# HpWang-whu/RoReg

Hardware: AMD Instinct MI355X
Metric: pair-registrations/sec (higher is better)
Workload: dtype f32 (every f32 operand enters the fp16 matrix cores as hi + lo fp16 under a per-keypoint power-of-two block scale: <= 22 significant bits relative to a CONSERVATIVE per-keypoint bound -- measured on the extractor: the bound sits 2^2..2^6 above the keypoint's true coefficient maximum (config.f16x2_sc

## Files before the change

include/roreg_hip.h:

```cpp
#ifndef ROREG_HIP_H
#define ROREG_HIP_H

#include <stdint.h>
#include <stddef.h>

#ifdef __cplusplus
extern "C" {
#endif

#define ROREG_ABI_VERSION 6
int roreg_abi_version(void);
const char *roreg_last_error(void);

int roreg_set_group_tables(const int32_t *P_host, const int32_t *Nei_host, const double *R_host);

size_t roreg_group_conv_packed_size(int Cin, int Cout, int KS);
int roreg_group_conv_pack_weights(const float *W_host , int Cin, int Cout, int KS,
                                  float *wpack_host );
size_t roreg_group_conv_workspace_size(int B, int Cin, int Cout, int Lin, int Lout, int KS);
int roreg_group_conv(const float *x, const float *wpack, const float *bias,
                     const float *bn_scale, const float *bn_shift, const float *residual,
                     float *out, const int32_t *gather,
                     int B, int Cin, int Cout, int Lin, int Lout, int KS,
                     float *workspace, size_t workspace_floats, void *stream);
// ... 217 lines not shown
int roreg_irrep_gemm(const float *const *X, float *const *Out, const float *const *Add, const float *const *Wpack, int C, int O, int B,
                     const int32_t *tiles_dev, int n_tiles, void *stream);
int roreg_irrep_gemm_split(const float *const *X, float *const *Out, const float *const *Add, const void *const *Wsplit, int C, int O, int B,
                           const int32_t *tiles_dev, int n_tiles, void *stream);
int roreg_irrep_gemm_f16x2(const float *const *X, float *const *Out, const float *const *Add, const void *const *Wsplit2,
                           const float *x_bound_dev, int w_exp, const float *next_u_dev, const float *next_v_dev, float *out_bound_dev,
                           int C, int O, int B, const int32_t *tiles_dev, int n_tiles,
                           int tile_m ,
                           int x_planes , void *stream);
int roreg_gemm_persistent(int on);
int roreg_gemm_thin(int on);
int roreg_irrep_gemm_f16x2_rows(const float *const *X, float *T3r, const void *const *Wsplit2, const float *x_bound_dev, int w_exp, int C, int B, void *stream);
int roreg_gf_finish(const float *T3r, const float *x, const float *b_out, const float *role_scale , const float *role_shift ,
                    float *eqv, float *inv, float *role_out , float *eqv_ft, int B, void *stream);
int roreg_gf_finish_route(int on);
int roreg_row_bound(const void *x_spatial, int x_bf16 , const float *bn_scale, const float *bn_shift,
                    float *bound_out, int B, int C, void *stream);
int roreg_ft_nonlin(const float *Xin , const float *x_spatial, const float *bias,
                    const float *bias2, const float *bn_scale, const float *bn_shift, const float *resid_spatial,
                    float *Xout , float *out_spatial ,
                    const int32_t *g_map ,
                    int Lout , int Lvalid,
                    int B, int C, int split ,
                    const float *out_bound ,
                    float *out_rowmax ,
                    int spatial_bf16 ,
                    int out_planes ,
                    void *stream);
int roreg_ft_nonlin_packed(const float *Xin, const float *bias, const float *bn_scale, const float *bn_shift, uint32_t *out_words,
                           const int32_t *g_map, int Lout, int Lvalid, int B, int C, const float *out_bound, float *raw_col, int raw_g,
// ... 210 lines not shown
```

roreg_amd/_abi.py:

```python
import ctypes
from ctypes import c_int, c_void_p, c_size_t, c_double, c_float, c_char_p

import numpy as np

ABI_VERSION = 6

_P = c_void_p
PROTOTYPES = {
    'roreg_abi_version': (c_int, []),
    'roreg_last_error': (c_char_p, []),
    'roreg_set_group_tables': (c_int, [_P, _P, _P]),
    'roreg_group_conv_packed_size': (c_size_t, [c_int, c_int, c_int]),
    'roreg_group_conv_pack_weights': (c_int, [_P, c_int, c_int, c_int, _P]),
    'roreg_group_conv_workspace_size': (c_size_t, [c_int, c_int, c_int, c_int, c_int, c_int]),
    'roreg_group_conv': (c_int, [_P, _P, _P, _P, _P, _P, _P, _P, c_int, c_int, c_int, c_int, c_int, c_int, _P, c_size_t, _P]),
    'roreg_group_conv_split': (c_int, [_P, _P, _P, _P, _P, _P, _P, _P, c_int, c_int, c_int, c_int, c_int, c_int, c_int, _P]),
    'roreg_group_conv_f16x2': (c_int, [_P, _P, c_int, _P, _P, _P, c_float, c_float, _P, _P, _P, _P, _P, c_int, c_int, c_int, c_int, c_int, c_int, c_int, _P]),
    'roreg_group_conv_f16x2_packed': (c_int, [_P, _P, c_int, _P, _P, _P, _P, _P, _P, c_int, c_int, c_int, c_int, c_int, c_int, c_int, _P]),
    'roreg_dense_f16x2': (c_int, [_P, _P, c_int, _P, _P, _P, c_float, c_float, _P, _P, c_int, _P, _P, c_int, c_int, c_int, _P]),
    'roreg_dense_split': (c_int, [_P, _P, _P, _P, _P, _P, c_int, _P, c_int, c_int, c_int, _P]),
    'roreg_gf_finalize': (c_int, [_P, _P, c_int, _P, c_int, _P]),
    'roreg_det_score': (c_int, [_P, _P, c_int, _P]),
    'roreg_inv_descriptor': (c_int, [_P, c_int, _P, c_int, _P]),
    'roreg_nn_search': (c_int, [_P, _P, c_int, _P, _P, c_int, c_int, _P, _P, _P, _P]),
# ... 42 lines not shown
    'roreg_sinkhorn_batch3_workspace_size': (c_size_t, [c_int, c_int, c_int, ctypes.c_longlong, ctypes.c_longlong, c_int, c_int]),
    'roreg_sinkhorn_batch3': (c_int, [_P, _P, _P, _P, _P, _P, _P, c_int, c_float, c_int, _P, _P, _P, _P, _P, c_size_t, c_int, _P, _P]),
    'roreg_write_files': (c_int, [_P, _P, _P, _P, _P, c_int, c_int]),
    'roreg_yohoc_draw_many': (c_int, [_P, c_int, _P, _P, c_int, c_int, _P, _P, _P, c_int]),
    'roreg_mlp_head_workspace': (c_size_t, [c_int, c_int, c_int]),
    'roreg_mlp_head': (c_int, [_P, _P, _P, _P, _P, c_int, c_int, c_int, c_int, _P, _P, c_int, _P, _P, _P, _P, _P, c_int, c_int, c_float, _P, _P, _P]),
    'roreg_sinkhorn_early_exit': (c_int, [c_int]),
    'roreg_sinkhorn_iteration_stats': (c_int, [_P, _P, c_int, _P]),
    'roreg_linear': (c_int, [_P, c_int, c_int, _P, _P, c_int, _P, _P]),
    'roreg_linear_mfma': (c_int, [_P, c_int, c_int, _P, _P, c_int, _P, _P]),
    'roreg_linear_path': (c_int, [c_int]),
    'roreg_linear_cat3': (c_int, [_P, _P, _P, _P, c_int, c_int, _P, _P, c_int, _P, _P]),
    'roreg_gemm_persistent': (c_int, [c_int]),
    'roreg_gemm_thin': (c_int, [c_int]),
    'roreg_gf_finish_route': (c_int, [c_int]),
    'roreg_irrep_gemm_f16x2_rows': (c_int, [_P, _P, _P, _P, c_int, c_int, c_int, _P]),
    'roreg_gf_finish': (c_int, [_P, _P, _P, _P, _P, _P, _P, _P, _P, c_int, _P]),
    'roreg_instnorm_stats': (c_int, [_P, c_int, c_int, c_float, _P, _P, _P, c_int, c_int, _P]),
    'roreg_mlp_tail': (c_int, [_P, c_int, c_int, _P, _P, _P, _P, _P, c_int, c_int, _P]),
    'roreg_mlp_tail_mfma': (c_int, [_P, c_int, c_int, _P, _P, _P, _P, _P, c_int, c_int, _P]),
    'roreg_knn_attention': (c_int, [_P, _P, _P, _P, c_int, c_int, c_int, c_int, _P, _P]),
    'roreg_rm_elementwise': (c_int, [c_int, _P, _P, _P, _P, c_int, c_int, c_int, _P, _P, _P]),
    'roreg_sinkhorn_workspace_size': (c_size_t, [c_int, c_int]),
    'roreg_sinkhorn': (c_int, [_P, c_int, _P, c_int, c_float, c_int, _P, _P, _P, _P, _P, _P, c_size_t, _P]),
    'roreg_icp_grid_size': (c_size_t, [_P, _P, c_int, c_double, _P, _P]),
    'roreg_icp_grid_build': (c_int, [_P, _P, _P, _P, c_size_t, _P]),
    'roreg_icp_batch_workspace': (c_size_t, [c_int, ctypes.c_longlong]),
    'roreg_icp_batch': (c_int, [_P, c_int, _P, c_int, ctypes.c_longlong, c_double, c_int, c_double, c_double, _P, _P, _P, _P, _P, _P, _P, _P, c_size_t, _P]),
    'roreg_icp_normals': (c_int, [_P, c_double, c_int, _P, _P]),
    'roreg_icp_plane_batch_workspace': (c_size_t, [c_int, ctypes.c_longlong]),
# ... 94 lines not shown
```

roreg_amd/_hip_fourier.py:

```python
import os
from ctypes import c_void_p

import numpy as np
import torch

from . import hip as _core
from .hip import HipError, _check, _feat, _ptr, _stream, lib

__all__ = ['DenseSplitLayer', 'IRREP_DIMS', 'IRREP_OFFSETS', '_bf16_split3', '_keypoint_of_columns', '_ptr_array', '_res_ptr', '_tile_cache', 'bf16_split3_frags', 'bf16_split3_pack', 'bound_exp', 'coef_pitch', 'coef_size', 'coef_views', 'dense_split', 'ensure_fourier', 'f16_scale_exp', 'f16_split2_frags', 'f16_split2_pack', 'frag_pack', 'ft_nonlin', 'ft_nonlin_gathered', 'ft_nonlin_packed', 'gemm_persistent', 'gemm_thin', 'gf_finish', 'gf_finish_rows', 'gf_finish_usable', 'group_conv_split_pack', 'irrep_gemm', 'irrep_gemm_rows', 'next_bound', 'next_bound_spatial', 'pack_coefs_f16x2', 'row_bound', 'unpack_coefs_f16x2', 'words_to_planes']


_fourier_ready = False
IRREP_DIMS = (1, 3, 3, 4, 5)
IRREP_OFFSETS = (0, 1, 10, 19, 35, 60)


def ensure_fourier():
    global _fourier_ready
    if not _fourier_ready:
        from .fourier import group_fourier
        F = np.ascontiguousarray(group_fourier().F, np.float32)
        _check(lib().roreg_set_fourier_tables(F.ctypes.data), 'roreg_set_fourier_tables')
        _fourier_ready = True

# ... 135 lines not shown
def row_bound(x, bn=None, roles=None):
    B, C = int(x.shape[0]), int(x.shape[1])
    out = torch.empty(coef_pitch(B), dtype=torch.float32, device=x.device)
    scale, shift = bn if bn is not None else (None, None)
    xp, bf = _feat(x)
    if roles is not None:
        if bn is not None or C != 32:
            raise HipError('row_bound: roles go with the 32-channel input features and no BatchNorm')
        r_scale, r_shift, role = _core._role_args(roles, B)
        _check(lib().roreg_row_bound_roles(xp, bf, _ptr(out), _ptr(r_scale), _ptr(r_shift), _ptr(role), B, _stream()), 'roreg_row_bound_roles')
        return out
    _check(lib().roreg_row_bound(xp, bf, _ptr(scale), _ptr(shift), _ptr(out), B, C, _stream()), 'roreg_row_bound')
    return out


def _keypoint_of_columns(d, Bp):
    n = torch.arange(d * Bp, device='cuda')
    return ((n // 32) // d) * 32 + (n % 32)


def bound_exp(bound):
    _, ex = torch.frexp(bound.float())
    e = torch.where((bound > 0) & torch.isfinite(bound), 14 - ex, torch.zeros_like(ex))
    return e.clamp(-100, 100)


def pack_coefs_f16x2(X_buf, C, B, bound=None):
    Bp = coef_pitch(B)
    views = coef_views(X_buf, C, B)
    if bound is None:
# ... 204 lines not shown
```

roreg_amd/csrc/fourier.hip:

```cpp
#include "common.h"
#include "primitives.h"
#include <algorithm>
#include <atomic>
#include <cmath>
#include <cstdlib>
#include <type_traits>
#include <utility>
#include <vector>

namespace {

constexpr int NIRR = 5;

struct GemmDescs {
    const float *X[NIRR];
    float *Out[NIRR];
    const float *Add[NIRR];
    const float4 *W[NIRR];
    int K[NIRR], M[NIRR], Mpad[NIRR], N[NIRR];
};

__device__ __forceinline__ void lds_dma16(const void *src, void *dst) {
    __builtin_amdgcn_global_load_lds((const __attribute__((address_space(1))) void *)src, (__attribute__((address_space(3))) void *)dst, 16, 0, 0);
}
// ... 1573 lines not shown
                t.qa[s] = off + l; t.row[s] = row0 + l; t.i[s] = 0; t.d[s] = d;
                if (l + 1 < d) { t.qb[s] = off + l + 1; t.kind[s] = 1; } else { t.qb[s] = 64; t.kind[s] = 2; }
            }
        off += d * d; row0 += d;
    }
    return t;
}
constexpr PairSlots kPS = make_pair_slots();
constexpr int slot_out_q(int m) { const int mm = m & 31, s = (m >> 5) * 16 + (mm & 3) + 4 * (mm >> 3); return (mm & 4) ? kPS.qb[s] : kPS.qa[s]; }

template <int... I, class F>
__device__ __forceinline__ void static_for_impl(std::integer_sequence<int, I...>, F &&f) { (f(std::integral_constant<int, I>{}), ...); }
template <int N, class F>
__device__ __forceinline__ void static_for(F &&f) { static_for_impl(std::make_integer_sequence<int, N>{}, f); }

template <bool IN_SPATIAL, bool OUT_SPATIAL, int SPLIT , int NW , int MINW , bool OUT_ROWS = false, bool GATHER = false >
__global__ __launch_bounds__(NW * 64, MINW) void ft_nonlin_kernel(NonlinParams p) {
    constexpr int NT = NW * 64;
    const int lane = threadIdx.x & 63;
    const int jn = lane & 31, h = lane >> 5;
    const int wave_global = __builtin_amdgcn_readfirstlane((blockIdx.x * NT + threadIdx.x) >> 6);
    const int n_waves = gridDim.x * NW;
    const int B = p.B, C = p.C;
    const int n_tiles = C * p.tiles_per_c;

    constexpr int NPL = SPLIT == 2 ? 2 : 3;
    constexpr int NA1 = SPLIT ? 4 * 2 * NPL * 64 * 4 : 30 * 2 * 64, NA2 = SPLIT ? 4 * 2 * NPL * 64 * 4 : 32 * 2 * 64;
    __shared__ __attribute__((aligned(16))) float sA1[IN_SPATIAL ? 64 : NA1];
    __shared__ __attribute__((aligned(16))) float sA2[OUT_SPATIAL ? 64 : NA2];
    __shared__ float sT[(IN_SPATIAL || OUT_SPATIAL || OUT_ROWS) ? NW * 32 * 65 : 64];
// ... 14 lines not shown
    for (int i = threadIdx.x; i < p.C; i += NT) {
        sBias[i] = (p.bias ? p.bias[i] : 0.f) + (p.bias2 ? p.bias2[i] : 0.f);
        sScale[i] = p.bn_scale ? p.bn_scale[i] : 1.f;
        sShift[i] = p.bn_shift ? p.bn_shift[i] : 0.f;
    }
    __syncthreads();
    const bf16x8 *sA1s = reinterpret_cast<const bf16x8 *>(sA1), *sA2s = reinterpret_cast<const bf16x8 *>(sA2);
    const f16x8 *sA1h = reinterpret_cast<const f16x8 *>(sA1), *sA2h = reinterpret_cast<const f16x8 *>(sA2);
    const size_t Bp = (size_t)p.Bp;
    const size_t hmask = (size_t)0 - (size_t)h;
#define OFF_Q(Q, c, tb) ((size_t)(kQ.alpha[Q] * C + (c) * kQ.d[Q]) * Bp + (size_t)(tb) * (32 * kQ.d[Q]) + kQ.i[Q] * 32)
#define OFF_OF(Q0, Q1, c, tb) (OFF_Q(Q0, c, tb) + ((OFF_Q(Q1, c, tb) - OFF_Q(Q0, c, tb)) & hmask))
    const unsigned lane_next = (unsigned)lane * 4u;
    const unsigned lane_row3 = (unsigned)jn * 4u + (h ? 12u * (unsigned)C * (unsigned)p.Bp : 0u);
    const unsigned lane_row5 = (unsigned)jn * 4u + (h ? 20u * (unsigned)C * (unsigned)p.Bp : 0u);
    auto row_off = [&](auto rc, int c, int tb) -> size_t {
        constexpr int R = decltype(rc)::value;
        return ((size_t)(kPS.row_alpha[R] * C) + (size_t)(c * kPS.row_d[R])) * Bp + (size_t)tb * (32 * kPS.row_d[R]);
    };
    auto slot_ptr = [&](auto sc, const void *buf, int c, int tb) -> const char * {
        constexpr int S = decltype(sc)::value;
        const char *rb = reinterpret_cast<const char *>(buf) + 4 * row_off(std::integral_constant<int, kPS.row[S]>{}, c, tb) + 128 * kPS.i[S];
        return rb + (kPS.kind[S] == 1 ? (kPS.d[S] == 3 ? lane_row3 : lane_row5) : lane_next);
    };

    constexpr int NCV = IN_SPATIAL ? 32 : (SPLIT != 0 ? 32 : 30);
    constexpr bool PACK_OUT = SPLIT == 2 && !OUT_SPATIAL && !OUT_ROWS;
    auto ld_sp = [&](const float *base, size_t i) -> float {
        return p.x_bf16 ? __uint_as_float((unsigned)reinterpret_cast<const unsigned short *>(base)[i] << 16) : base[i];
    };
    float cn[NCV + 1];
    struct GDesc { unsigned lo, hi; int a; };
    auto load_desc = [&](int tile) -> GDesc {
        GDesc d{0u, 0u, 0};
        if constexpr (GATHER) {
            const int c = tile % C, tb = tile / C;
            const int row = min(tb * 32 + jn, B - 1);
            const uint2 w = *reinterpret_cast<const uint2 *>(&p.g_rows[row].src[c >> 5]);
            d.lo = w.x; d.hi = w.y;
// ... 49 lines not shown
        } else if constexpr (SPLIT != 0) {
            static_for<32>([&](auto ic) {
                constexpr int st = decltype(ic)::value / 8, e = decltype(ic)::value % 8;
                constexpr int q0 = 16 * st + e, q1 = 16 * st + 8 + e;
                if constexpr (q1 < ROREG_G) dst[st * 8 + e] = __builtin_nontemporal_load(p.Xin + OFF_OF(q0, q1, c, tb) + jn);
                else dst[st * 8 + e] = __builtin_nontemporal_load(p.Xin + OFF_Q(q0, c, tb) + jn);
            });
        } else {
            static_for<30>([&](auto ic) {
                constexpr int s = decltype(ic)::value;
                constexpr int q0 = 2 * s, q1 = 2 * s + 1;
                dst[s] = p.Xin[OFF_OF(q0, q1, c, tb) + jn];
            });
        }
    };
    auto table_mma = [&](const auto *a, const auto (&b)[NPL], f32x16 c) {
        std::remove_cv_t<std::remove_reference_t<decltype(b[0])>> av[NPL];
#pragma unroll
        for (int pl = 0; pl < NPL; ++pl) av[pl] = a[64 * pl];
        return split_mma<NPL>(av, b, c);
    };
    auto column_scale = [&](float mx, float &xscale, float &oscale) {
        mx = fmaxf(mx, __shfl_xor(mx, 32));
        int e = 0;
        if (mx > 0.f && mx < __builtin_inff()) { int ex; (void)frexpf(mx, &ex); e = 14 - ex; }
        xscale = ldexpf(1.f, e); oscale = ldexpf(1.f, -(e + p.f_exp));
    };
    auto process = [&](int tile, int next_tile, float (&cv)[NCV + 1], float (&cnext)[NCV + 1], int next2_tile, const GDesc &dnext, GDesc &dnext2) {
        asm volatile("" ::: "memory");
        const int c = (IN_SPATIAL || OUT_SPATIAL) ? tile % C : tile / p.tiles_per_c;
        const int tbi = (IN_SPATIAL || OUT_SPATIAL) ? tile / C : tile - c * p.tiles_per_c;
        const int b = tbi * 32 + jn;
        const bool valid = b < B;
        const int bb = valid ? b : B - 1;
        f32x16 v[2];
        float wmax = 0.f;
        if (IN_SPATIAL) {
            if constexpr (GATHER) {
                dnext2 = load_desc(next2_tile);
                load_rows_gathered(next_tile, dnext, cnext);
            } else {
                load_coefs(next_tile, cnext);
// ... 63 lines not shown
        const float sc = sScale[c], sh = sShift[c];
        const bool has_rs = OUT_SPATIAL && p.r_spatial;
        const bool rs_late = has_rs && !bn && !p.g_map && !p.out_rowmax;
        const size_t rs = ((size_t)bb * C + c) * ROREG_G;
        float *tb = (OUT_SPATIAL || OUT_ROWS) ? sT + (threadIdx.x >> 6) * (32 * 65) : nullptr;
        const bool sp_pack = OUT_SPATIAL && SPLIT == 2 && p.sp_pack;
        const float pk_scale = sp_pack ? ldexpf(1.f, bound_exp(cv[NCV])) : 1.f;
#pragma unroll
        for (int t = 0; t < 2; ++t)
#pragma unroll
            for (int r = 0; r < 16; ++r) {
                const int g = t * 32 + (r & 3) + 8 * (r >> 2) + 4 * h;
                float x = v[t][r] + bsum;
                if (OUT_SPATIAL && has_rs && !rs_late && g < ROREG_G) x += ld_sp(p.r_spatial, rs + g);
                if (sp_pack && p.raw_col && g == p.raw_g && valid) p.raw_col[(size_t)bb * C + c] = x;
                if (bn) x = fmaxf(fmaf(x, sc, sh), 0.f);
                if (g >= ROREG_G || !valid) x = 0.f;
                v[t][r] = x;
                if (OUT_SPATIAL && g < ROREG_G) {
                    const int go = sGmap[g];
                    if (go >= 0) {
                        if (sp_pack) {
                            const float xs = x * pk_scale;
                            const _Float16 h1 = (_Float16)xs;
                            const _Float16 l1 = (_Float16)(xs - (float)h1);
                            tb[jn * 65 + go] = __uint_as_float((unsigned)__builtin_bit_cast(unsigned short, h1) | ((unsigned)__builtin_bit_cast(unsigned short, l1) << 16));
                        } else {
                            tb[jn * 65 + go] = x; wmax = fmaxf(wmax, fabsf(x));
                        }
                    }
                }
// ... 207 lines not shown

    auto load = [&](int b, float (&cv)[32], float (&xv)[32]) {
        const float *t = p.T3r + (size_t)b * (ROREG_G * ROREG_F) + h * (8 * ROREG_F) + jn;
        static_for<32>([&](auto ic) {
            constexpr int st = decltype(ic)::value / 8, e = decltype(ic)::value % 8;
            constexpr int q0 = 16 * st + e, q1 = 16 * st + 8 + e;
            if constexpr (q1 < ROREG_G) cv[st * 8 + e] = __builtin_nontemporal_load(t + q0 * ROREG_F);
            else cv[st * 8 + e] = __builtin_nontemporal_load(t + q0 * ROREG_F - h * (8 * ROREG_F));
        });
        const float *xs = p.x + (size_t)b * (ROREG_F * ROREG_G) + (act ? lane : 0);
        static_for<32>([&](auto ic) {
            constexpr int c = decltype(ic)::value;
            xv[c] = xs[c * ROREG_G];
        });
    };
    auto table_mma = [&](const f16x8 *a, const f16x8 (&b)[2], f32x16 c) {
        f16x8 av[2];
#pragma unroll
        for (int pl = 0; pl < 2; ++pl) av[pl] = a[64 * pl];
        return split_mma<2>(av, b, c);
    };
    auto column_scale = [&](float mx, float &xscale, float &oscale) {
        mx = fmaxf(mx, __shfl_xor(mx, 32));
        int e = 0;
        if (mx > 0.f && mx < __builtin_inff()) { int ex; (void)frexpf(mx, &ex); e = 14 - ex; }
        xscale = ldexpf(1.f, e); oscale = ldexpf(1.f, -(e + p.f_exp));
    };
    auto transform = [&](const f16x8 *tab, const float (&k)[32], f32x16 (&v)[2]) {
        float mx = 0.f;
#pragma unroll
        for (int s = 0; s < 32; ++s) mx = fmaxf(mx, fabsf(k[s]));
        float xsc, osc;
        column_scale(mx, xsc, osc);
#pragma unroll
        for (int t = 0; t < 2; ++t)
#pragma unroll
            for (int r = 0; r < 16; ++r) v[t][r] = 0.f;
#pragma unroll
        for (int st = 0; st < 4; ++st) {
            float x8[8];
#pragma unroll
            for (int e = 0; e < 8; ++e) x8[e] = k[st * 8 + e];
// ... 111 lines not shown
        }
        ROREG_LDS_DONE();
    };
#undef ROREG_LDS_DONE
    if (wave_global < B) {
        const int last = wave_global + ((B - 1 - wave_global) / n_waves) * n_waves;
        float ca[32], xa[32], cb[32], xb[32];
        load(wave_global, ca, xa);
        __builtin_amdgcn_s_waitcnt(0x0F70);
        for (int b = wave_global; b <= last; b += 2 * n_waves) {
            const int b1 = min(b + n_waves, last), b2 = min(b + 2 * n_waves, last);
            process(b, b1, ca, xa, cb, xb);
            process(b1, b2, cb, xb, ca, xa);
        }
    }
}

float *g_A1 = nullptr, *g_A2 = nullptr;
uint16_t *g_A1s = nullptr, *g_A2s = nullptr, *g_A1h = nullptr, *g_A2h = nullptr;
int g_f_exp = 0;

}

extern "C" int roreg_set_fourier_tables(const float *F_host ) {
    ROREG_REQUIRE(F_host, "roreg_set_fourier_tables: null table");
    static float A1[30 * 2 * 64], A2[32 * 2 * 64];
    for (int s = 0; s < 30; ++s)
        for (int tile = 0; tile < 2; ++tile)
            for (int lane = 0; lane < 64; ++lane) {
                const int qq = 2 * s + (lane >> 5), g = tile * 32 + (lane & 31);
// ... 167 lines not shown
        }
        return x;
    }
    int set(int on) {
        const int prev = get();
        if (on >= 0 && on <= hi) v.store(on, std::memory_order_relaxed);
        return prev;
    }
};
static GemmSwitch g_gemm_persist{"ROREG_GEMM_PERSIST", 0, 2};
static GemmSwitch g_gf_finish{"ROREG_GF_FINISH", 1, 1};
static GemmSwitch g_gemm_thin{"ROREG_GEMM_THIN", 1, 1};
extern "C" int roreg_gemm_persistent(int on) { return g_gemm_persist.set(on); }
extern "C" int roreg_gemm_thin(int on) { return g_gemm_thin.set(on); }
extern "C" int roreg_gf_finish_route(int on) { return g_gf_finish.set(on); }
static int gemm_cu_count() {
    static const int n = [] {
        int dev = 0, cus = 0;
        if (hipGetDevice(&dev) != hipSuccess || hipDeviceGetAttribute(&cus, hipDeviceAttributeMultiprocessorCount, dev) != hipSuccess || cus <= 0) cus = 256;
        return cus;
    }();
    return n;
}
template <int NP, int WO>
static int launch_gemm_split(const char *what, const float *const *X, float *const *Out, const float *const *Add, const void *const *Wsplit,
                             const float *xbound, int w_exp, const float *nb_u, const float *nb_v, float *out_bound, int C, int O, int B,
                             const int32_t *tiles_dev, int n_tiles, void *stream, int x_planes = 0) {
    static const int dims[5] = {1, 3, 3, 4, 5};
    GemmSplitDescs p;
    for (int r = 0; r < 5; ++r) {
// ... 116 lines not shown
    hipLaunchKernelGGL(row_bound_roles_kernel, dim3((Bp + 3) / 4), dim3(256), 0, roreg::as_stream(stream), reinterpret_cast<const float *>(x_spatial), x_bf16, bound_out,
                       B, Bp, role_scale, role_shift, role_out);
    ROREG_CHECK_LAUNCH("roreg_row_bound_roles");
    return 0;
}

extern "C" int roreg_row_bound(const void *x_spatial, int x_bf16, const float *bn_scale, const float *bn_shift, float *bound_out, int B, int C,
                               void *stream) {
    ROREG_REQUIRE(x_spatial && bound_out && B > 0 && C > 0, "roreg_row_bound: bad arguments");
    ROREG_REQUIRE((bn_scale == nullptr) == (bn_shift == nullptr), "roreg_row_bound: bn_scale and bn_shift go together");
    const int Bp = (B + 31) / 32 * 32;
    hipLaunchKernelGGL(row_bound_kernel, dim3((Bp + 3) / 4), dim3(256), 0, roreg::as_stream(stream), reinterpret_cast<const float *>(x_spatial), x_bf16, bn_scale, bn_shift,
                       bound_out, B, Bp, C);
    ROREG_CHECK_LAUNCH("roreg_row_bound");
    return 0;
}

template <void (*KERN)(NonlinParams)>
static void launch_ft(const NonlinParams &p, long long n_tiles, hipStream_t s) {
    static const int resident = [] {
        int per_cu = 0, dev = 0, cus = 256;
        if (hipOccupancyMaxActiveBlocksPerMultiprocessor(&per_cu, KERN, 256, 0) != hipSuccess || per_cu < 1) per_cu = 2;
        if (hipGetDevice(&dev) == hipSuccess) (void)hipDeviceGetAttribute(&cus, hipDeviceAttributeMultiprocessorCount, dev);
        return per_cu * cus;
    }();
    static const int rounds = [] { const char *e = getenv("ROREG_FT_ROUNDS"); const int r = e ? atoi(e) : 0; return r > 0 ? r : 4; }();
    const long long want = (n_tiles + 3) / 4, cap = (long long)resident * rounds;
    hipLaunchKernelGGL(KERN, dim3((unsigned)(want > cap ? cap : want)), dim3(256), 0, s, p);
}

// ... 154 lines not shown
```

roreg_amd/network/gf_fourier.py:

```python
import numpy as np
import torch

from .. import hip
from ..fourier import group_fourier, DIMS
from .ops import _version_key


def _fold_bn(bn):
    scale = bn.weight.detach().float().cpu() / torch.sqrt(bn.running_var.detach().float().cpu() + bn.eps)
    shift = bn.bias.detach().float().cpu() - bn.running_mean.detach().float().cpu() * scale
    return scale.cuda().contiguous(), shift.cuda().contiguous()


class _Layer:
    def __init__(self, conv):
        gf = group_fourier()
        W = conv.weight.detach().double().cpu().numpy()
        O, C = W.shape[0], W.shape[1]
        W = W.reshape(O, C, 13)
        self.C, self.O = C, O
        self.bias = conv.bias.detach().float().cuda().contiguous()
        self.wpack = []
        self.wsplit = []
        self.dense = []
# ... 27 lines not shown
            self._key = key

    def _plan_bounds(self):
        if getattr(self, '_nb_key', None) != self._key:
            self.nb_1 = hip.next_bound(self.bn_1, self.l_in.bias)
            self.nb_2 = hip.next_bound(self.bn_2, self.l_1.bias)
            self.nb_3 = hip.next_bound(self.bn_3, self.l_2.bias, self.l_in.bias)
            self._nb_key = self._key

    def _conv_out_operand(self, x, roles=None):
        self._plan()
        hip.ensure_fourier()
        B = x.shape[0]
        sp = 'f16x2'
        self._plan_bounds()
        b0 = hip.row_bound(x, roles=roles)
        X0 = hip.ft_nonlin(B, 32, x_spatial=x, split=sp, out_bound=b0)
        T0, b1 = hip.irrep_gemm(X0, None, 32, 256, B, f16x2=self.l_in.wsplit2, x_bound=b0, next_bound=self.nb_1)
        del X0
        xd = hip.use_planes(512) and hip.use_planes(256)
        X1 = hip.ft_nonlin(B, 256, coef_in=T0, bias=self.l_in.bias, bn=self.bn_1, split=sp, out_bound=b1, planes=xd)
        T1, b2 = hip.irrep_gemm(X1, None, 256, 512, B, f16x2=self.l_1.wsplit2, x_bound=b1, next_bound=self.nb_2, x_planes=xd)
        del X1
        X2 = hip.ft_nonlin(B, 512, coef_in=T1, bias=self.l_1.bias, bn=self.bn_2, split=sp, out_bound=b2, planes=xd)
        del T1
        T2, b3 = hip.irrep_gemm(X2, None, 512, 256, B, f16x2=self.l_2.wsplit2, x_bound=b2, next_bound=self.nb_3, add=T0, x_planes=xd)
        del X2, T0
        return hip.ft_nonlin(B, 256, coef_in=T2, bias=self.l_2.bias, bias2=self.l_in.bias, bn=self.bn_3, split=sp, out_bound=b3), b3

    def forward_finished(self, x, roles=None):
        if self.gemm != 'f16x2' or x.dtype != torch.float32:
            raise hip.HipError('FourierGF.forward_finished: the fp16 x 2 mode on float32 features only')
# ... 75 lines not shown
            b = self.block
            self.l_in = _Layer(b.comb_layer_in[2]); self.bn_in = _fold_bn(b.comb_layer_in[0])
            self.l_out = _Layer(b.comb_layer_out[2]); self.bn_out = _fold_bn(b.comb_layer_out[0])
            self.l_sc = _Layer(b.short_cut_layer[2]); self.bn_sc = _fold_bn(b.short_cut_layer[0])
            self._key = key

    def forward(self, x):
        self._plan()
        hip.ensure_fourier()
        B = x.shape[0]
        sp = {'f32': False, 'bf16x3': True, 'f16x2': 'f16x2'}[self.gemm]
        if self.gemm == 'f16x2':
            if getattr(self, '_nb_key', None) != self._key:
                self.nb_out = hip.next_bound(self.bn_out, self.l_in.bias)
                self._nb_key = self._key
            bs = hip.row_bound(x, bn=self.bn_sc)
            Xs = hip.ft_nonlin(B, 32, x_spatial=x, bn=self.bn_sc, split=sp, out_bound=bs)
            S = hip.irrep_gemm(Xs, None, self.l_sc.C, self.l_sc.O, B, f16x2=self.l_sc.wsplit2, x_bound=bs)
            del Xs
            ba = hip.row_bound(x, bn=self.bn_in)
            Xa = hip.ft_nonlin(B, 32, x_spatial=x, bn=self.bn_in, split=sp, out_bound=ba)
            T1, b1 = hip.irrep_gemm(Xa, None, self.l_in.C, self.l_in.O, B, f16x2=self.l_in.wsplit2, x_bound=ba, next_bound=self.nb_out)
            del Xa
            X1 = hip.ft_nonlin(B, 64, coef_in=T1, bias=self.l_in.bias, bn=self.bn_out, split=sp, out_bound=b1)
            del T1
            T2 = hip.irrep_gemm(X1, None, self.l_out.C, self.l_out.O, B, f16x2=self.l_out.wsplit2, x_bound=b1, add=S)
            del X1, S
            return hip.ft_nonlin(B, 16, coef_in=T2, bias=self.l_out.bias, bias2=self.l_sc.bias, spatial_out=True, split=sp)

        def gemm(X, layer, add=None):
            return hip.irrep_gemm(X, layer.wpack, layer.C, layer.O, B, split=layer.wsplit if self.gemm == 'bf16x3' else None, add=add)

        def ft(C, **kw):
            return hip.ft_nonlin(B, C, split=sp, **kw)
        Xs = ft(32, x_spatial=x, bn=self.bn_sc)
        S = gemm(Xs, self.l_sc)
# ... 10 lines not shown
```

Baseline: 1132.

## Fuse row-bound and spatial Fourier transform into one-pass head kernel

After: 1135, median of 6. No clear change (+0.2%).

```diff
diff --git a/include/roreg_hip.h b/include/roreg_hip.h
--- a/include/roreg_hip.h
+++ b/include/roreg_hip.h
@@ -255,6 +255,9 @@
 int roreg_gf_finish(const float *T3r, const float *x, const float *b_out, const float *role_scale , const float *role_shift ,
                     float *eqv, float *inv, float *role_out , float *eqv_ft, int B, void *stream);
 int roreg_gf_finish_route(int on);
+int roreg_gf_head(const float *x, const float *bn_scale, const float *bn_shift, const float *role_scale, const float *role_shift, float *role_out,
+                  float *bound_out, float *Xout, int B, void *stream);
+int roreg_gf_head_route(int on);
 int roreg_row_bound(const void *x_spatial, int x_bf16 , const float *bn_scale, const float *bn_shift,
                     float *bound_out, int B, int C, void *stream);
 int roreg_ft_nonlin(const float *Xin , const float *x_spatial, const float *bias,
diff --git a/roreg_amd/_abi.py b/roreg_amd/_abi.py
--- a/roreg_amd/_abi.py
+++ b/roreg_amd/_abi.py
@@ -80,6 +80,8 @@
     'roreg_gemm_persistent': (c_int, [c_int]),
     'roreg_gemm_thin': (c_int, [c_int]),
     'roreg_gf_finish_route': (c_int, [c_int]),
+    'roreg_gf_head_route': (c_int, [c_int]),
+    'roreg_gf_head': (c_int, [_P, _P, _P, _P, _P, _P, _P, _P, c_int, _P]),
     'roreg_irrep_gemm_f16x2_rows': (c_int, [_P, _P, _P, _P, c_int, c_int, c_int, _P]),
     'roreg_gf_finish': (c_int, [_P, _P, _P, _P, _P, _P, _P, _P, _P, c_int, _P]),
     'roreg_instnorm_stats': (c_int, [_P, c_int, c_int, c_float, _P, _P, _P, c_int, c_int, _P]),
diff --git a/roreg_amd/_hip_fourier.py b/roreg_amd/_hip_fourier.py
--- a/roreg_amd/_hip_fourier.py
+++ b/roreg_amd/_hip_fourier.py
@@ -7,7 +7,7 @@
 from . import hip as _core
 from .hip import HipError, _check, _feat, _ptr, _stream, lib
 
-__all__ = ['DenseSplitLayer', 'IRREP_DIMS', 'IRREP_OFFSETS', '_bf16_split3', '_keypoint_of_columns', '_ptr_array', '_res_ptr', '_tile_cache', 'bf16_split3_frags', 'bf16_split3_pack', 'bound_exp', 'coef_pitch', 'coef_size', 'coef_views', 'dense_split', 'ensure_fourier', 'f16_scale_exp', 'f16_split2_frags', 'f16_split2_pack', 'frag_pack', 'ft_nonlin', 'ft_nonlin_gathered', 'ft_nonlin_packed', 'gemm_persistent', 'gemm_thin', 'gf_finish', 'gf_finish_rows', 'gf_finish_usable', 'group_conv_split_pack', 'irrep_gemm', 'irrep_gemm_rows', 'next_bound', 'next_bound_spatial', 'pack_coefs_f16x2', 'row_bound', 'unpack_coefs_f16x2', 'words_to_planes']
+__all__ = ['DenseSplitLayer', 'IRREP_DIMS', 'IRREP_OFFSETS', '_bf16_split3', '_keypoint_of_columns', '_ptr_array', '_res_ptr', '_tile_cache', 'bf16_split3_frags', 'bf16_split3_pack', 'bound_exp', 'coef_pitch', 'coef_size', 'coef_views', 'dense_split', 'ensure_fourier', 'f16_scale_exp', 'f16_split2_frags', 'f16_split2_pack', 'frag_pack', 'ft_nonlin', 'ft_nonlin_gathered', 'ft_nonlin_packed', 'gemm_persistent', 'gemm_thin', 'ft_head', 'gf_finish', 'gf_finish_rows', 'gf_finish_usable', 'gf_head', 'gf_head_usable', 'group_conv_split_pack', 'irrep_gemm', 'irrep_gemm_rows', 'next_bound', 'next_bound_spatial', 'pack_coefs_f16x2', 'row_bound', 'unpack_coefs_f16x2', 'words_to_planes']
 
 
 _fourier_ready = False
@@ -173,6 +173,31 @@
     return out
 
 
+gf_head = _GemmSwitch('roreg_gf_head_route', lambda on: int(bool(on)),
+                      """`with hip.gf_head(True | False):` -- whether the extractor and the detector open with the one-pass head (ft_head, gf_head_kernel; roreg_gf_head_route;
+    the default, ROREG_GF_HEAD=0 in the environment turns it off) or with row_bound + ft_nonlin.  Same bits either way -- tests and A/B measurements.""")
+
+
+def gf_head_usable(gemm_mode, x):
+    return gemm_mode == 'f16x2' and x.dtype == torch.float32 and tuple(x.shape[1:]) == (32, 60) and lib().roreg_gf_head_route(-1) == 1
+
+
+def ft_head(x, bn=None, roles=None):
+    ensure_fourier()
+    B = int(x.shape[0])
+    if tuple(x.shape[1:]) != (32, 60) or x.dtype != torch.float32:
+        raise HipError('ft_head: x [B,32,60] float32')
+    bound = torch.empty(coef_pitch(B), dtype=torch.float32, device=x.device)
+    out = torch.empty(coef_size(32, B), dtype=torch.float32, device=x.device)
+    scale, shift = bn if bn is not None else (None, None)
+    r_scale = r_shift = role = None
+    if roles is not None:
+        r_scale, r_shift, role = _core._role_args(roles, B)
+    _check(lib().roreg_gf_head(_ptr(x, torch.float32), _ptr(scale), _ptr(shift), _ptr(r_scale), _ptr(r_shift), _ptr(role), _ptr(bound), _ptr(out), B, _stream()),
+           'roreg_gf_head')
+    return out, bound
+
+
 def _keypoint_of_columns(d, Bp):
     n = torch.arange(d * Bp, device='cuda')
     return ((n // 32) // d) * 32 + (n % 32)
diff --git a/roreg_amd/csrc/fourier.hip b/roreg_amd/csrc/fourier.hip
--- a/roreg_amd/csrc/fourier.hip
+++ b/roreg_amd/csrc/fourier.hip
@@ -1611,6 +1611,68 @@
 template <int N, class F>
 __device__ __forceinline__ void static_for(F &&f) { static_for_impl(std::make_integer_sequence<int, N>{}, f); }
 
+template <int NPL, class F>
+__device__ __forceinline__ f32x16 ft_table_mma(const F *a, const F (&b)[NPL], f32x16 c) {
+    F av[NPL];
+#pragma unroll
+    for (int pl = 0; pl < NPL; ++pl) av[pl] = a[64 * pl];
+    return split_mma<NPL>(av, b, c);
+}
+__device__ __forceinline__ void ft_column_scale(float mx, int f_exp, float &xscale, float &oscale) {
+    mx = fmaxf(mx, __shfl_xor(mx, 32));
+    int e = 0;
+    if (mx > 0.f && mx < __builtin_inff()) { int ex; (void)frexpf(mx, &ex); e = 14 - ex; }
+    xscale = ldexpf(1.f, e); oscale = ldexpf(1.f, -(e + f_exp));
+}
+__device__ __forceinline__ float ft_transform_f16x2(const f16x8 *tab, int lane, int f_exp, const float (&k)[32], f32x16 (&v)[2]) {
+    float mx = 0.f;
+#pragma unroll
+    for (int s = 0; s < 32; ++s) mx = fmaxf(mx, fabsf(k[s]));
+    float xsc, osc;
+    ft_column_scale(mx, f_exp, xsc, osc);
+#pragma unroll
+    for (int t = 0; t < 2; ++t)
+#pragma unroll
+        for (int r = 0; r < 16; ++r) v[t][r] = 0.f;
+#pragma unroll
+    for (int st = 0; st < 4; ++st) {
+        float x8[8];
+#pragma unroll
+        for (int e = 0; e < 8; ++e) x8[e] = k[st * 8 + e];
+        f16x8 bh, bl;
+        split2(x8, xsc, bh, bl);
+        const f16x8 b[2] = {bh, bl};
+        v[0] = ft_table_mma<2>(tab + ((st * 2 + 0) * 2) * 64 + lane, b, v[0]);
+        v[1] = ft_table_mma<2>(tab + ((st * 2 + 1) * 2) * 64 + lane, b, v[1]);
+    }
+    return osc;
+}
+__device__ __forceinline__ float split_word(float x) {
+    const _Float16 h1 = (_Float16)x;
+    const _Float16 l1 = (_Float16)(x - (float)h1);
+    return __uint_as_float((unsigned)__builtin_bit_cast(unsigned short, h1) | ((unsigned)__builtin_bit_cast(unsigned short, l1) << 16));
+}
+struct SlotLanes {
+    unsigned next, row3, row5;
+};
+template <int R>
+__device__ __forceinline__ size_t slot_row_off(int C, size_t Bp, int c, int tb) {
+    return ((size_t)(kPS.row_alpha[R] * C) + (size_t)(c * kPS.row_d[R])) * Bp + (size_t)tb * (32 * kPS.row_d[R]);
+}
+template <int S>
+__device__ __forceinline__ const char *slot_addr(const void *buf, int C, size_t Bp, int c, int tb, const SlotLanes &l) {
+    const char *rb = reinterpret_cast<const char *>(buf) + 4 * slot_row_off<kPS.row[S]>(C, Bp, c, tb) + 128 * kPS.i[S];
+    return rb + (kPS.kind[S] == 1 ? (kPS.d[S] == 3 ? l.row3 : l.row5) : l.next);
+}
+__device__ __forceinline__ void ft_store_slots(float *Xout, int C, size_t Bp, int c, int tb, int h, const SlotLanes &l, const f32x16 (&o)[2]) {
+    static_for<32>([&](auto ic) {
+        constexpr int S = decltype(ic)::value, t = S / 16, r = S % 16;
+        float *dst = reinterpret_cast<float *>(const_cast<char *>(slot_addr<S>(Xout, C, Bp, c, tb, l)));
+        if (kPS.kind[S] != 2 || h == 0) __builtin_nontemporal_store(o[t][r], dst);
+    });
+}
+__device__ __forceinline__ float bn_relu(float x, float sc, float sh) { return fmaxf(fmaf(x, sc, sh), 0.f); }
+
 template <bool IN_SPATIAL, bool OUT_SPATIAL, int SPLIT , int NW , int MINW , bool OUT_ROWS = false, bool GATHER = false >
 __global__ __launch_bounds__(NW * 64, MINW) void ft_nonlin_kernel(NonlinParams p) {
     constexpr int NT = NW * 64;
@@ -1655,15 +1717,8 @@
     const unsigned lane_next = (unsigned)lane * 4u;
     const unsigned lane_row3 = (unsigned)jn * 4u + (h ? 12u * (unsigned)C * (unsigned)p.Bp : 0u);
     const unsigned lane_row5 = (unsigned)jn * 4u + (h ? 20u * (unsigned)C * (unsigned)p.Bp : 0u);
-    auto row_off = [&](auto rc, int c, int tb) -> size_t {
-        constexpr int R = decltype(rc)::value;
-        return ((size_t)(kPS.row_alpha[R] * C) + (size_t)(c * kPS.row_d[R])) * Bp + (size_t)tb * (32 * kPS.row_d[R]);
-    };
-    auto slot_ptr = [&](auto sc, const void *buf, int c, int tb) -> const char * {
-        constexpr int S = decltype(sc)::value;
-        const char *rb = reinterpret_cast<const char *>(buf) + 4 * row_off(std::integral_constant<int, kPS.row[S]>{}, c, tb) + 128 * kPS.i[S];
-        return rb + (kPS.kind[S] == 1 ? (kPS.d[S] == 3 ? lane_row3 : lane_row5) : lane_next);
-    };
+    const SlotLanes slot_lanes{lane_next, lane_row3, lane_row5};
+    auto slot_ptr = [&](auto sc, const void *buf, int c, int tb) -> const char * { return slot_addr<decltype(sc)::value>(buf, C, Bp, c, tb, slot_lanes); };
 
     constexpr int NCV = IN_SPATIAL ? 32 : (SPLIT != 0 ? 32 : 30);
     constexpr bool PACK_OUT = SPLIT == 2 && !OUT_SPATIAL && !OUT_ROWS;
@@ -1743,18 +1798,8 @@
             });
         }
     };
-    auto table_mma = [&](const auto *a, const auto (&b)[NPL], f32x16 c) {
-        std::remove_cv_t<std::remove_reference_t<decltype(b[0])>> av[NPL];
-#pragma unroll
-        for (int pl = 0; pl < NPL; ++pl) av[pl] = a[64 * pl];
-        return split_mma<NPL>(av, b, c);
-    };
-    auto column_scale = [&](float mx, float &xscale, float &oscale) {
-        mx = fmaxf(mx, __shfl_xor(mx, 32));
-        int e = 0;
-        if (mx > 0.f && mx < __builtin_inff()) { int ex; (void)frexpf(mx, &ex); e = 14 - ex; }
-        xscale = ldexpf(1.f, e); oscale = ldexpf(1.f, -(e + p.f_exp));
-    };
+    auto table_mma = [&](const auto *a, const auto (&b)[NPL], f32x16 c) { return ft_table_mma<NPL>(a, b, c); };
+    auto column_scale = [&](float mx, float &xscale, float &oscale) { ft_column_scale(mx, p.f_exp, xscale, oscale); };
     auto process = [&](int tile, int next_tile, float (&cv)[NCV + 1], float (&cnext)[NCV + 1], int next2_tile, const GDesc &dnext, GDesc &dnext2) {
         asm volatile("" ::: "memory");
         const int c = (IN_SPATIAL || OUT_SPATIAL) ? tile % C : tile / p.tiles_per_c;
@@ -1848,7 +1893,7 @@
                 float x = v[t][r] + bsum;
                 if (OUT_SPATIAL && has_rs && !rs_late && g < ROREG_G) x += ld_sp(p.r_spatial, rs + g);
                 if (sp_pack && p.raw_col && g == p.raw_g && valid) p.raw_col[(size_t)bb * C + c] = x;
-                if (bn) x = fmaxf(fmaf(x, sc, sh), 0.f);
+                if (bn) x = bn_relu(x, sc, sh);
                 if (g >= ROREG_G || !valid) x = 0.f;
                 v[t][r] = x;
                 if (OUT_SPATIAL && g < ROREG_G) {
@@ -2086,18 +2131,8 @@
             xv[c] = xs[c * ROREG_G];
         });
     };
-    auto table_mma = [&](const f16x8 *a, const f16x8 (&b)[2], f32x16 c) {
-        f16x8 av[2];
-#pragma unroll
-        for (int pl = 0; pl < 2; ++pl) av[pl] = a[64 * pl];
-        return split_mma<2>(av, b, c);
-    };
-    auto column_scale = [&](float mx, float &xscale, float &oscale) {
-        mx = fmaxf(mx, __shfl_xor(mx, 32));
-        int e = 0;
-        if (mx > 0.f && mx < __builtin_inff()) { int ex; (void)frexpf(mx, &ex); e = 14 - ex; }
-        xscale = ldexpf(1.f, e); oscale = ldexpf(1.f, -(e + p.f_exp));
-    };
+    auto table_mma = [&](const f16x8 *a, const f16x8 (&b)[2], f32x16 c) { return ft_table_mma<2>(a, b, c); };
+    auto column_scale = [&](float mx, float &xscale, float &oscale) { ft_column_scale(mx, p.f_exp, xscale, oscale); };
     auto transform = [&](const f16x8 *tab, const float (&k)[32], f32x16 (&v)[2]) {
         float mx = 0.f;
 #pragma unroll
@@ -2239,6 +2274,150 @@
             process(b1, b2, cb, xb, ca, xa);
         }
     }
+}
+
+struct GfHeadParams {
+    const float *x;
+    const float *bn_scale, *bn_shift;
+    const float *role_scale, *role_shift;
+    float *role_out;
+    float *bound;
+    float *Xout;
+    const f16x8 *A2h;
+    int f_exp, B, Bp;
+};
+constexpr int kHeadTable = 4 * 2 * 2 * 64 * 4;
+constexpr int kHeadWaves = 16;
+constexpr size_t kHeadLds = (size_t)(kHeadTable + kHeadWaves * 32 * 65 + 2 * 3 * kHeadWaves * 32 + 192) * sizeof(float);
+
+__global__ __launch_bounds__(1024) void gf_head_kernel(GfHeadParams p) {
+    constexpr int NW = kHeadWaves, NT = NW * 64;
+    extern __shared__ __attribute__((aligned(16))) float gh_smem[];
+    float *sA2 = gh_smem, *sT = sA2 + kHeadTable;
+    float *sRed = sT + NW * 32 * 65;
+    float *sCh = sRed + 2 * 3 * NW * 32;
+    const int lane = threadIdx.x & 63, jn = lane & 31, h = lane >> 5;
+    const int wave = __builtin_amdgcn_readfirstlane((int)threadIdx.x >> 6);
+    {
+        const float *g2 = reinterpret_cast<const float *>(p.A2h);
+        for (int i = threadIdx.x; i < kHeadTable; i += NT) sA2[i] = g2[i];
+        const int i = threadIdx.x;
+        if (i < 32) sCh[i] = p.bn_scale ? p.bn_scale[i] : 1.f;
+        else if (i < 64) sCh[i] = p.bn_shift ? p.bn_shift[i - 32] : 0.f;
+        else if (i < 128) sCh[i] = p.role_scale ? p.role_scale[i - 64] : 0.f;
+        else if (i < 192) sCh[i] = p.role_shift ? p.role_shift[i - 128] : 0.f;
+    }
+    __syncthreads();
+    const f16x8 *sA2h = reinterpret_cast<const f16x8 *>(sA2);
+    const bool bn = p.bn_scale != nullptr, roles = p.role_scale != nullptr;
+    const int B = p.B, n_tiles = p.Bp >> 5;
+    const size_t Bp = (size_t)p.Bp;
+    const SlotLanes slot_lanes{(unsigned)lane * 4u, (unsigned)jn * 4u + (h ? 12u * (unsigned)ROREG_F * (unsigned)p.Bp : 0u),
+                               (unsigned)jn * 4u + (h ? 20u * (unsigned)ROREG_F * (unsigned)p.Bp : 0u)};
+    float *ti = sT + wave * (32 * 65);
+    const unsigned xl = lane < ROREG_G ? lane : 0;
+    const int c0 = wave * 2;
+#define ROREG_LDS_DONE() asm volatile("s_waitcnt lgkmcnt(0)" ::: "memory")
+    int parity = 0;
+    for (int tb = blockIdx.x; tb < n_tiles; tb += gridDim.x, parity ^= 1) {
+        const int b0 = tb * 32;
+        const bool valid = b0 + jn < B;
+        float cv[2][32];
+        static_for<64>([&](auto ic) {
+            constexpr int k = decltype(ic)::value / 32, i = decltype(ic)::value % 32;
+            const float *row = p.x + ((size_t)(b0 + i < B ? b0 + i : B - 1) * ROREG_F + (c0 + k)) * ROREG_G;
+            cv[k][i] = row[xl];
+        });
+        __builtin_amdgcn_sched_barrier(0);
+        asm volatile("" ::: "memory");
+        auto read_tile = [&](float (&k)[32]) {
+#pragma unroll
+            for (int s = 0; s < 32; ++s) {
+                const int g = cd_row32(s & 15, h, (s >> 4) * 32);
+                k[s] = g < ROREG_G ? ti[jn * 65 + g] : 0.f;
+            }
+            ROREG_LDS_DONE();
+        };
+        auto activate = [&](float (&k)[32], int c) {
+            const float sc = sCh[c], sh = sCh[32 + c];
+#pragma unroll
+            for (int s = 0; s < 32; ++s) {
+                float xg = k[s] + 0.f;
+                if (bn) xg = bn_relu(xg, sc, sh);
+                if (cd_row32(s & 15, h, (s >> 4) * 32) >= ROREG_G || !valid) xg = 0.f;
+                k[s] = xg;
+            }
+        };
+        float mxk = 0.f, m1 = 0.f, m0 = 0.f;
+        auto maxima = [&](float (&k)[32], int c) {
+            if (roles) {
+                const float s1 = sCh[64 + c], s0 = sCh[96 + c], h1 = sCh[128 + c], h0 = sCh[160 + c];
+#pragma unroll
+                for (int s = 0; s < 32; ++s)
+                    if (cd_row32(s & 15, h, (s >> 4) * 32) < ROREG_G) {
+                        m1 = fmaxf(m1, fmaxf(fmaf(k[s], s1, h1), 0.f));
+                        m0 = fmaxf(m0, fmaxf(fmaf(k[s], s0, h0), 0.f));
+                    }
+            }
+            activate(k, c);
+#pragma unroll
+            for (int s = 0; s < 32; ++s) mxk = fmaxf(mxk, fabsf(k[s]));
+        };
+        float k0[32];
+        {
+#pragma unroll
+            for (int i = 0; i < 32; ++i) ti[i * 65 + lane] = cv[0][i];
+            ROREG_LDS_DONE();
+            read_tile(k0);
+            maxima(k0, c0);
+            __builtin_amdgcn_sched_barrier(0);
+#pragma unroll
+            for (int i = 0; i < 32; ++i) ti[i * 65 + lane] = cv[1][i];
+            ROREG_LDS_DONE();
+            float k1[32];
+            read_tile(k1);
+            maxima(k1, c0 + 1);
+        }
+        mxk = fmaxf(mxk, __shfl_xor(mxk, 32)); m1 = fmaxf(m1, __shfl_xor(m1, 32)); m0 = fmaxf(m0, __shfl_xor(m0, 32));
+        float *red = sRed + parity * (3 * NW * 32);
+        if (h == 0) { red[wave * 32 + jn] = mxk; red[(NW + wave) * 32 + jn] = m1; red[(2 * NW + wave) * 32 + jn] = m0; }
+        __syncthreads();
+        float mx = 0.f;
+#pragma unroll
+        for (int w = 0; w < NW; ++w) mx = fmaxf(mx, red[w * 32 + jn]);
+        const float bound = mx * 7.7536f;
+        if (wave == 0 && h == 0) {
+            p.bound[b0 + jn] = bound;
+            if (roles && valid) {
+                float r1 = 0.f, r0 = 0.f;
+#pragma unroll
+                for (int w = 0; w < NW; ++w) { r1 = fmaxf(r1, red[(NW + w) * 32 + jn]); r0 = fmaxf(r0, red[(2 * NW + w) * 32 + jn]); }
+                p.role_out[(size_t)(b0 + jn) * 4] = r1; p.role_out[(size_t)(b0 + jn) * 4 + 1] = r0;
+            }
+        }
+        ROREG_LDS_DONE();
+        const float bscale = ldexpf(1.f, bound_exp(bound));
+        auto finish = [&](const float (&k)[32], int c) {
+            asm volatile("" : "+s"(c));
+            f32x16 o[2];
+            const float osc = ft_transform_f16x2(sA2h, lane, p.f_exp, k, o);
+            const float psc = osc * bscale;
+#pragma unroll
+            for (int t = 0; t < 2; ++t)
+#pragma unroll
+                for (int r = 0; r < 16; ++r) o[t][r] = split_word(o[t][r] * psc);
+            ft_store_slots(p.Xout, ROREG_F, Bp, c, tb, h, slot_lanes, o);
+        };
+        finish(k0, c0);
+        __builtin_amdgcn_sched_barrier(0);
+        {
+            float k1[32];
+            read_tile(k1);
+            activate(k1, c0 + 1);
+            finish(k1, c0 + 1);
+        }
+    }
+#undef ROREG_LDS_DONE
 }
 
 float *g_A1 = nullptr, *g_A2 = nullptr;
@@ -2436,6 +2615,8 @@
 extern "C" int roreg_gemm_persistent(int on) { return g_gemm_persist.set(on); }
 extern "C" int roreg_gemm_thin(int on) { return g_gemm_thin.set(on); }
 extern "C" int roreg_gf_finish_route(int on) { return g_gf_finish.set(on); }
+static GemmSwitch g_gf_head{"ROREG_GF_HEAD", 1, 1};
+extern "C" int roreg_gf_head_route(int on) { return g_gf_head.set(on); }
 static int gemm_cu_count() {
     static const int n = [] {
         int dev = 0, cus = 0;
@@ -2582,6 +2763,25 @@
                        bound_out, B, Bp, C);
     ROREG_CHECK_LAUNCH("roreg_row_bound");
     return 0;
+}
+
+extern "C" int roreg_gf_head(const float *x, const float *bn_scale, const float *bn_shift, const float *role_scale, const float *role_shift, float *role_out,
+                             float *bound_out, float *Xout, int B, void *stream) {
+    ROREG_REQUIRE(g_A2h, "roreg_gf_head: roreg_set_fourier_tables has not been called");
+    ROREG_REQUIRE(x && bound_out && Xout && B > 0, "roreg_gf_head: bad arguments");
+    ROREG_REQUIRE((bn_scale == nullptr) == (bn_shift == nullptr), "roreg_gf_head: bn_scale and bn_shift go together");
+    ROREG_REQUIRE((role_scale == nullptr) == (role_shift == nullptr) && (role_scale == nullptr) == (role_out == nullptr),
+                  "roreg_gf_head: role_scale, role_shift and role_out go together");
+    GfHeadParams p;
+    memset(&p, 0, sizeof(p));
+    p.x = x; p.bn_scale = bn_scale; p.bn_shift = bn_shift; p.role_scale = role_scale; p.role_shift = role_shift; p.role_out = role_out;
+    p.bound = bound_out; p.Xout = Xout; p.A2h = reinterpret_cast<const f16x8 *>(g_A2h); p.f_exp = g_f_exp;
+    p.B = B; p.Bp = (B + 31) / 32 * 32;
+    ROREG_REQUIRE((unsigned long long)ROREG_F * p.Bp * 20ull < (1ull << 32), "roreg_gf_head: 32 * round_up(B, 32) must stay below 2^32 / 20 (32-bit lane offsets)");
+    hipStream_t s = roreg::as_stream(stream);
+    roreg::ProfScope prof(roreg::PROF_FT_NONLIN, s);
+    const int n_tiles = p.Bp / 32;
+    return roreg::launch_lds("roreg_gf_head", gf_head_kernel, dim3((unsigned)std::min(n_tiles, gemm_cu_count())), dim3(kHeadWaves * 64), kHeadLds, s, p);
 }
 
 template <void (*KERN)(NonlinParams)>
diff --git a/roreg_amd/network/gf_fourier.py b/roreg_amd/network/gf_fourier.py
--- a/roreg_amd/network/gf_fourier.py
+++ b/roreg_amd/network/gf_fourier.py
@@ -65,8 +65,11 @@
         B = x.shape[0]
         sp = 'f16x2'
         self._plan_bounds()
-        b0 = hip.row_bound(x, roles=roles)
-        X0 = hip.ft_nonlin(B, 32, x_spatial=x, split=sp, out_bound=b0)
+        if hip.gf_head_usable('f16x2', x):
+            X0, b0 = hip.ft_head(x, roles=roles)
+        else:
+            b0 = hip.row_bound(x, roles=roles)
+            X0 = hip.ft_nonlin(B, 32, x_spatial=x, split=sp, out_bound=b0)
         T0, b1 = hip.irrep_gemm(X0, None, 32, 256, B, f16x2=self.l_in.wsplit2, x_bound=b0, next_bound=self.nb_1)
         del X0
         xd = hip.use_planes(512) and hip.use_planes(256)
@@ -172,12 +175,19 @@
             if getattr(self, '_nb_key', None) != self._key:
                 self.nb_out = hip.next_bound(self.bn_out, self.l_in.bias)
                 self._nb_key = self._key
-            bs = hip.row_bound(x, bn=self.bn_sc)
-            Xs = hip.ft_nonlin(B, 32, x_spatial=x, bn=self.bn_sc, split=sp, out_bound=bs)
+            head = hip.gf_head_usable('f16x2', x)
+            if head:
+                Xs, bs = hip.ft_head(x, bn=self.bn_sc)
+            else:
+                bs = hip.row_bound(x, bn=self.bn_sc)
+                Xs = hip.ft_nonlin(B, 32, x_spatial=x, bn=self.bn_sc, split=sp, out_bound=bs)
             S = hip.irrep_gemm(Xs, None, self.l_sc.C, self.l_sc.O, B, f16x2=self.l_sc.wsplit2, x_bound=bs)
             del Xs
-            ba = hip.row_bound(x, bn=self.bn_in)
-            Xa = hip.ft_nonlin(B, 32, x_spatial=x, bn=self.bn_in, split=sp, out_bound=ba)
+            if head:
+                Xa, ba = hip.ft_head(x, bn=self.bn_in)
+            else:
+                ba = hip.row_bound(x, bn=self.bn_in)
+                Xa = hip.ft_nonlin(B, 32, x_spatial=x, bn=self.bn_in, split=sp, out_bound=ba)
             T1, b1 = hip.irrep_gemm(Xa, None, self.l_in.C, self.l_in.O, B, f16x2=self.l_in.wsplit2, x_bound=ba, next_bound=self.nb_out)
             del Xa
             X1 = hip.ft_nonlin(B, 64, coef_in=T1, bias=self.l_in.bias, bn=self.bn_out, split=sp, out_bound=b1)
```
